# natir/yacrd

Measured on AMD Instinct MI355X. Metric: reads_per_sec_classified, higher is better.
Workload: dtype u32

## Files before the change

yacrd_amd/csrc/device_common.h:

```cpp
#pragma once
#include <hip/hip_runtime.h>
#include <stdint.h>

typedef uint32_t u32;
typedef uint64_t u64;
typedef int32_t i32;

namespace yk {

constexpr u32 kNoKey = 0xFFFFFFFFu;

typedef u32 u32x4_a8 __attribute__((ext_vector_type(4), aligned(8)));
template <bool NT = false>
__device__ __forceinline__ uint4 load_pair(const uint2 *p)
{
    u32x4_a8 q;
    if constexpr (NT) q = __builtin_nontemporal_load(reinterpret_cast<const u32x4_a8 *>(p));
    else q = *reinterpret_cast<const u32x4_a8 *>(p);
    return make_uint4(q.x, q.y, q.z, q.w);
}
typedef u64 u64x2_a8 __attribute__((ext_vector_type(2), aligned(8)));
__device__ __forceinline__ ulonglong2 load_extent(const u64 *p)
{
    const u64x2_a8 q = *reinterpret_cast<const u64x2_a8 *>(p);
    return make_ulonglong2(q.x, q.y);
}

struct OvlRec {
    u32 a, b, sa, ea, sb, eb;
};

constexpr u32 kKeyShift = 2;
constexpr u32 kMaxKeyPos = 0x3FFFFFFEu;
__device__ __forceinline__ void make_event_keys(uint2 v, u32 &ks, u32 &ke, u32 &bad, u32 &zero_len)
{
    const u32 z = (v.x == v.y) ? 2u : 0u;
    bad |= (v.x > v.y || v.y > kMaxKeyPos) ? 1u : 0u;
    zero_len += z;
    ks = ((v.x << kKeyShift) | 3u) - z;
    ke = (v.y << kKeyShift) + z;
}
constexpr u32 kNoFlag = 1u;

constexpr u32 kSmallEvents = 1024;
constexpr u32 kMedium1Events = 8192;
constexpr u32 kMedium2Events = 32768;
enum { CLS_R2 = 0, CLS_R4, CLS_R8, CLS_R16, CLS_H16, CLS_W2, CLS_W4, CLS_W8, CLS_W16, CLS_MED1,
       CLS_MED2, CLS_GENERAL, CLS_COUNT };

struct Counters {
    u32 n[16];
    u64 iv[16];
    u32 rej_small;
    u32 rej_med;
    u32 rej_big;
    u32 region_overflow;
    u32 scan_ticket;
    u32 ob_unsupported;
    u32 prefiltered;
    u32 over_med;
    u32 fb_med[2];
    u32 fb_big;
    u32 fbq_head[2];
    u32 fbq_done[2];
    u32 bs_chunks;
    u32 fused_gave_up;
    u64 total_regions;
    u32 fb_stream[2];
    alignas(128) u32 deferred;
    u64 deferred_iv;
};

struct SweepArgs {
    const u64 *off;
    const uint2 *iv;
    const u32 *len;
    const u32 *list;
    const u32 *list_n;
    const uint4 *rec;
    u32 first;
    u32 cov;
    u32 prefilter;
    uint2 *stage;
    u32 *counts;
    uint2 *closed;
    u32 *rej_list;
    u32 *rej_count;
    u32 *over_list;
    u32 *over_count;
    Counters *ctr;
};
constexpr u32 kDeferredMark = 0xFFFFFFFFu;
constexpr u32 kClosedForm = 0xFFFFFFFEu;

__device__ __forceinline__ u32 lane_id() { return threadIdx.x & 63u; }

#define YK_DPP_ZERO(v, ctrl, rm) (u32) __builtin_amdgcn_update_dpp(0, (int)(v), ctrl, rm, 0xF, true)
__device__ __forceinline__ u32 wave_incl_add(u32 v)
{
    v += YK_DPP_ZERO(v, 0x111, 0xF);
    v += YK_DPP_ZERO(v, 0x112, 0xF);
    v += YK_DPP_ZERO(v, 0x114, 0xF);
    v += YK_DPP_ZERO(v, 0x118, 0xF);
    v += YK_DPP_ZERO(v, 0x142, 0xA);
    v += YK_DPP_ZERO(v, 0x143, 0xC);
    return v;
}
__device__ __forceinline__ u32 wave_incl_max(u32 v)
{
    v = max(v, YK_DPP_ZERO(v, 0x111, 0xF));
    v = max(v, YK_DPP_ZERO(v, 0x112, 0xF));
    v = max(v, YK_DPP_ZERO(v, 0x114, 0xF));
    v = max(v, YK_DPP_ZERO(v, 0x118, 0xF));
    v = max(v, YK_DPP_ZERO(v, 0x142, 0xA));
    v = max(v, YK_DPP_ZERO(v, 0x143, 0xC));
    return v;
}
__device__ __forceinline__ u32 wave_shift_up1(u32 v) { return YK_DPP_ZERO(v, 0x138, 0xF); }
__device__ __forceinline__ u32 wave_min(u32 v)
{
#pragma unroll
    for (u32 d = 32; d > 0; d >>= 1) v = min(v, (u32)__shfl_xor(v, d, 64));
    return v;
}
__device__ __forceinline__ u32 wave_max(u32 v)
{
#pragma unroll
    for (u32 d = 32; d > 0; d >>= 1) v = max(v, (u32)__shfl_xor(v, d, 64));
    return v;
}
__device__ __forceinline__ u32 wave_or(u32 v)
{
#pragma unroll
    for (u32 d = 32; d > 0; d >>= 1) v |= (u32)__shfl_xor(v, d, 64);
    return v;
}

template <int T>
__device__ __forceinline__ u32 block_excl_add(u32 v, u32 *sc, u32 &total)
{
    u32 incl = wave_incl_add(v);
    if (T == 64) {
        total = __shfl(incl, 63, 64);
        return incl - v;
    }
    const u32 wid = threadIdx.x >> 6;
    if (lane_id() == 63) sc[wid] = incl;
    __syncthreads();
    u32 base = 0, tot = 0;
#pragma unroll
    for (u32 w = 0; w < T / 64; w++) {
        u32 x = sc[w];
        if (w < wid) base += x;
        tot += x;
// ... 89 lines not shown
```

yacrd_amd/csrc/finish_compact.h:

```cpp
#pragma once
#include "plan_compact.h"
#include "screen_reg.h"
#include "sweep_filtered.h"
#include "sweep_lds.h"
#include "sweep_wave.h"
#include "wave_ops.h"

namespace yk {

struct CompactArgs2 {
    SweepArgs sweep;
    u64 *scan_state;
    u32 n_reads;
    double not_cov;
    u64 *bad_offsets;
    uint2 *bad_regions;
    u64 region_cap;
    uint8_t *read_type;
    Counters *host_ctr;
};

constexpr int kFinishWaves = kScanBlock / 64;
#ifndef YK_FINISH_OCC
#define YK_FINISH_OCC 8
// ... 102 lines not shown
            for (i32 hi = (i32)bid - 1;; hi -= 64) {
                const i32 idx = hi - (i32)lane;
                u64 v, pre;
                for (;;) {
                    v = idx >= 0 ? __hip_atomic_load(&c.scan_state[idx], __ATOMIC_RELAXED, __HIP_MEMORY_SCOPE_AGENT)
                                 : kPre;
                    pre = __builtin_amdgcn_ballot_w64((v >> 62) == 2);
                    const u64 before = pre ? ((pre & (0 - pre)) - 1ull) : ~0ull;
                    if ((__builtin_amdgcn_ballot_w64((v >> 62) == 0) & before) == 0) break;
                    __builtin_amdgcn_s_sleep(1);
                }
                const u32 first_pre = pre ? (u32)__builtin_ctzll(pre) : 64u;
                u64 part = lane <= first_pre ? (v & kVal) : 0;
#pragma unroll
                for (int d = 32; d > 0; d >>= 1) part += __shfl_xor(part, d, 64);
                base += part;
                if (pre) break;
            }
        }
        if (lane == 0) {
            __hip_atomic_store(&c.scan_state[bid], kPre | (base + tot), __ATOMIC_RELAXED, __HIP_MEMORY_SCOPE_AGENT);
            s_base = base;
            if ((u64)(bid + 1) * kScanBlock >= c.n_reads) ctr->total_regions = base + tot;
        }
        if (c.host_ctr && (u64)(bid + 1) * kScanBlock >= c.n_reads) {
            const u64 total = (u64)__shfl((long long)(base + tot), 0, 64);
            const u32 *src = reinterpret_cast<const u32 *>(ctr);
            u32 *dst = reinterpret_cast<u32 *>(c.host_ctr);
            constexpr u32 kWords = (u32)(sizeof(Counters) / 4);
            for (u32 i = lane; i < kWords; i += 64u) {
                u32 w = __hip_atomic_load(&src[i], __ATOMIC_RELAXED, __HIP_MEMORY_SCOPE_AGENT);
                if (i == (u32)(offsetof(Counters, total_regions) / 4)) w = (u32)total;
                if (i == (u32)(offsetof(Counters, total_regions) / 4) + 1u) w = (u32)(total >> 32);
                if (i == (u32)(offsetof(Counters, region_overflow) / 4)) w = total > c.region_cap ? 1u : 0u;
                dst[i] = w;
            }
        }
    }
    __syncthreads();
    if (in) {
        const u64 dst = s_base + local;
        c.bad_offsets[r] = dst;
        if (r == c.n_reads - 1) c.bad_offsets[c.n_reads] = dst + g;

        u32 bad = 0;
        bool middle = false;
        const bool fits = dst + g <= c.region_cap;
        if (closed) {
            u32 k = 0;
            if (ab.x != 0u && fits) c.bad_regions[dst + k++] = make_uint2(0u, ab.x);
            if (ab.y != L && fits) c.bad_regions[dst + k] = make_uint2(ab.y, L);
            bad = ab.x + (L - ab.y);
        } else {
            const uint2 *slot = a.stage + (off_r + 2 * (u64)r);
            for (u32 k = 0; k < g; k++) {
                const uint2 v = slot[k];
                if (fits) c.bad_regions[dst + k] = v;
                bad += v.y - v.x;
                middle |= (v.x != 0u) & (v.y != L);
            }
        }
        if (!fits) atomicOr(&ctr->region_overflow, 1u);
        c.read_type[r] = (uint8_t)classify(bad, middle, L, c.not_cov);
    }
}


#ifndef YK_DEFER_SWEEP_OCC
#define YK_DEFER_SWEEP_OCC 6
#endif

template <int LANES, int WPB, int TABW = kScreenTabWords>
__device__ __forceinline__ bool filtered_turn(const SweepArgs &a, bool active, u32 r, u64 o, u32 n, u32 len, const LaneConst &lc)
{
    constexpr int K = 16;
    const u32 lane = lane_id(), lig = lane & (u32)(LANES - 1);
    const i32 c = (i32)min(a.cov, 0x3FFFFFFFu);
    const bool two = active && n >= 2u;
    const uint2 *src = two ? a.iv + o : reinterpret_cast<const uint2 *>(a.off);
    const u32 last2 = two ? n - 2u : 0u;
    uint4 v[K / 4];
#pragma unroll
    for (int j = 0; j < K / 4; j++) v[j] = load_pair(src + min(2u * (lig + (u32)LANES * j), last2));
    u32 smin = v[0].x, emax = v[0].y, smax = v[0].x;
    i32 tmin = 0x7FFFFFFF;
#pragma unroll
    for (int j = 0; j < K / 4; j++) {
        smin = min(smin, min(v[j].x, v[j].z));
        smax = max(smax, max(v[j].x, v[j].z));
        emax = max(emax, max(v[j].y, v[j].w));
        tmin = min(tmin, min((i32)(v[j].y - v[j].x), (i32)(v[j].w - v[j].z)));
    }
    const int last_addr = (int)((lane | (u32)(LANES - 1)) << 2);
    const u32 pmin = (u32)__builtin_amdgcn_ds_bpermute(last_addr, (int)gscan_min<LANES>(smin));
    const u32 pmax = (u32)__builtin_amdgcn_ds_bpermute(last_addr, (int)gscan_max<LANES>(emax));
    const bool irregular = !two || pmax > min(len, kMaxKeyPos) || smax > kMaxKeyPos || tmin < (i32)kScreenWindow;
    const bool girr = group_any<LANES>(__builtin_amdgcn_ballot_w64(irregular));
    const u32 n_eff = girr ? 0u : n;
    bool real0[K / 4], real1[K / 4];
#pragma unroll
    for (int j = 0; j < K / 4; j++) {
        const u32 i0 = 2u * (lig + (u32)LANES * j);
        real0[j] = i0 + 1u < n_eff;
        real1[j] = i0 < n_eff;
    }
    return filtered_group_sweep<LANES, WPB, TABW>(a, v, real0, real1, r, o, n, len, c, pmin, pmax, !girr, lc);
}
constexpr u32 kDeferShards = 256, kDeferShardStride = 16;
struct DeferList {
    u32 *list;
    u32 *count;
    u32 shard_cap;
};
constexpr int kMarkThreads = 1024, kMarkReads = 4 * kMarkThreads;
__global__ __launch_bounds__(kMarkThreads) void mark_list_kernel(const u32 *__restrict__ counts, u32 n_reads, DeferList dl)
{
    __shared__ u32 s_ids[kMarkReads];
    __shared__ u32 s_n, s_base;
    if (threadIdx.x == 0) s_n = 0;
    __syncthreads();
    const u64 r0 = (u64)blockIdx.x * kMarkReads + threadIdx.x * 4u;
    u32 g[4] = {0, 0, 0, 0};
    if (r0 + 4 <= n_reads) {
        const uint4 g4 = *reinterpret_cast<const uint4 *>(counts + r0);
        g[0] = g4.x, g[1] = g4.y, g[2] = g4.z, g[3] = g4.w;
    } else {
#pragma unroll
        for (int k = 0; k < 4; k++) g[k] = r0 + k < n_reads ? counts[r0 + k] : 0u;
    }
    u32 mine = 0;
#pragma unroll
    for (int k = 0; k < 4; k++) mine += g[k] == kDeferredMark ? 1u : 0u;
    if (__builtin_amdgcn_ballot_w64(mine != 0) != 0) {
        u32 incl = mine;
#pragma unroll
        for (int d = 1; d < 64; d <<= 1) {
            const u32 t = (u32)__shfl_up((int)incl, d, 64);
            if ((int)lane_id() >= d) incl += t;
        }
        u32 base = 0;
        if (lane_id() == 63u) base = atomicAdd(&s_n, incl);
        base = (u32)__shfl((int)base, 63, 64);
        u32 at = base + incl - mine;
#pragma unroll
        for (int k = 0; k < 4; k++)
            if (g[k] == kDeferredMark) s_ids[at++] = (u32)(r0 + k);
    }
    __syncthreads();
    const u32 n = s_n;
    if (n == 0) return;
    const u32 shard = blockIdx.x & (kDeferShards - 1u);
    if (threadIdx.x == 0) s_base = atomicAdd(dl.count + shard * kDeferShardStride, n);
    __syncthreads();
    const u32 b0 = s_base;
    for (u32 i = threadIdx.x; i < n; i += kMarkThreads)
        if (b0 + i < dl.shard_cap) dl.list[(size_t)shard * dl.shard_cap + b0 + i] = s_ids[i];
}

#ifndef YK_LIST_THREADS
#define YK_LIST_THREADS 512
#endif
#ifndef YK_LIST_OCC
#define YK_LIST_OCC YK_DEFER_SWEEP_OCC
#endif
constexpr int kListThreads = YK_LIST_THREADS;
__global__ __launch_bounds__(kListThreads, YK_LIST_OCC) void deferred_list_kernel(SweepArgs a, DeferList dl)
{
    constexpr u32 kWaves = kListThreads / 64;
    constexpr int kTabWords = 2 * (2 * kScreenWindow + 32) * 4;
    static_assert(kDeferShards <= (u32)kListThreads, "one thread per shard counter");
    __shared__ u32 s_pre[kDeferShards + 1];
    __shared__ u32 sc[kWaves + 1];
    __shared__ uint4 s_list[kListThreads];
    __shared__ unsigned short s_fb[kListThreads];
    __shared__ u32 s_nfb;
    __shared__ unsigned long long s_iv;
    const u32 tid = threadIdx.x, lane = lane_id(), wv = tid >> 6;
    u32 total;
    {
        const u32 cnt = tid < kDeferShards ? min(dl.count[tid * kDeferShardStride], dl.shard_cap) : 0u;
        const u32 ex = block_excl_add<kListThreads>(cnt, sc, total);
        if (tid < kDeferShards) s_pre[tid] = ex;
        if (tid == 0) s_pre[kDeferShards] = total;
    }
    const u32 per = (total + gridDim.x - 1u) / gridDim.x;
    const u32 lo = (u32)min((u64)total, (u64)blockIdx.x * per), hi = (u32)min((u64)total, (u64)lo + per);
    if (lo >= hi) return;
    const LaneConst lcf = make_lane_const(lane);
    if (tid == 0) s_iv = 0;
    for (u32 c0 = lo; c0 < hi; c0 += (u32)kListThreads) {
        __syncthreads();
        if (tid == 0) s_nfb = 0;
        const u32 e = c0 + tid, n_here = min((u32)kListThreads, hi - c0);
        if (e < hi) {
            u32 s = 0;
#pragma unroll
            for (u32 step = kDeferShards / 2; step > 0; step >>= 1)
                if (s_pre[s + step] <= e) s += step;
            const u32 r = dl.list[(size_t)s * dl.shard_cap + (e - s_pre[s])];
            const u64 o = a.off[r];
            const u32 n = (u32)(a.off[r + 1] - o);
            s_list[tid] = make_uint4(r, n, a.len[r], 0u);
            atomicAdd(&s_iv, (unsigned long long)n);
        }
        __syncthreads();
        for (u32 p0 = wv * 2u; p0 < n_here; p0 += kWaves * 2u) {
            const u32 p = p0 + (lane >> 5);
            const bool have = p < n_here;
            const uint4 q = s_list[have ? p : p0];
            const u64 o = a.off[q.x];
            const bool done = filtered_turn<32, (int)kWaves, kTabWords>(a, have, q.x, o, q.y, q.z, lcf);
            if (have && !done && (lane & 31u) == 31u) s_fb[atomicAdd(&s_nfb, 1u)] = (unsigned short)p;
        }
        __syncthreads();
        const u32 nfb = s_nfb;
        for (u32 i = wv; i < nfb; i += kWaves) {
            const uint4 q = s_list[s_fb[i]];
            const u64 o = a.off[q.x];
            if (q.y > 128u) finish_item<8>(a.off, a.iv, a.len, a.stage, a.counts, a.rej_list, a.rej_count, a.ctr, a.cov, q.x, o, q.y, q.z);
            else finish_item<4>(a.off, a.iv, a.len, a.stage, a.counts, a.rej_list, a.rej_count, a.ctr, a.cov, q.x, o, q.y, q.z);
        }
    }
    __syncthreads();
    if (tid == 0) {
        atomicAdd((unsigned long long *)&a.ctr->deferred_iv, s_iv);
        atomicAdd(&a.ctr->deferred, hi - lo);
    }
}

constexpr int kScanThreads = 1024;
template <int PER>
__global__ __launch_bounds__(kScanThreads) void scan_compact_kernel(CompactArgs2 c)
{
    constexpr int kScanPer = PER, kScanReads = kScanThreads * PER;
    static_assert(PER % 4 == 0 && kScanReads % kScanBlock == 0, "16-byte loads; the control block holds one scan word per 1024 reads: more than this kernel's workgroups use");
    __shared__ u32 sc[kScanThreads / 64];
    __shared__ u32 s_bid;
    __shared__ u64 s_base;
    const SweepArgs &a = c.sweep;
    Counters *ctr = a.ctr;
    if (threadIdx.x == 0) s_bid = atomicAdd(&ctr->scan_ticket, 1u);
    __syncthreads();
    const u32 bid = s_bid, lane = lane_id();
    const u64 r0 = (u64)bid * kScanReads + threadIdx.x * (u32)kScanPer;
    u32 g[kScanPer], L[kScanPer];
    uint2 ab[kScanPer];
    bool closed[kScanPer];
    const bool vec = r0 + kScanPer <= c.n_reads && (reinterpret_cast<uintptr_t>(a.len) & 15u) == 0;
    if (vec) {
#pragma unroll
        for (int q = 0; q < kScanPer / 4; q++) {
            const uint4 g4 = *reinterpret_cast<const uint4 *>(a.counts + r0 + 4 * q);
            const uint4 l4 = *reinterpret_cast<const uint4 *>(a.len + r0 + 4 * q);
            g[4 * q] = g4.x, g[4 * q + 1] = g4.y, g[4 * q + 2] = g4.z, g[4 * q + 3] = g4.w;
            L[4 * q] = l4.x, L[4 * q + 1] = l4.y, L[4 * q + 2] = l4.z, L[4 * q + 3] = l4.w;
        }
    } else {
#pragma unroll
        for (int k = 0; k < kScanPer; k++) {
            const bool in = r0 + k < c.n_reads;
            g[k] = in ? a.counts[r0 + k] : 0u;
            L[k] = in ? a.len[r0 + k] : 0u;
        }
    }
    bool any_closed = false;
#pragma unroll
    for (int k = 0; k < kScanPer; k++) {
        if (g[k] == kDeferredMark) g[k] = 0u;
        closed[k] = g[k] == kClosedForm;
        any_closed |= closed[k];
        ab[k] = make_uint2(0u, L[k]);
    }
    if (any_closed) {
        if (vec) {
#pragma unroll
            for (int q = 0; q < kScanPer / 2; q++) {
                const uint4 c0 = *reinterpret_cast<const uint4 *>(a.closed + r0 + 2 * q);
                if (closed[2 * q]) ab[2 * q] = make_uint2(c0.x, c0.y);
                if (closed[2 * q + 1]) ab[2 * q + 1] = make_uint2(c0.z, c0.w);
            }
        } else {
#pragma unroll
            for (int k = 0; k < kScanPer; k++)
                if (closed[k]) ab[k] = a.closed[r0 + k];
        }
    }
    u32 mine = 0;
#pragma unroll
    for (int k = 0; k < kScanPer; k++) {
        if (closed[k]) g[k] = (ab[k].x != 0u ? 1u : 0u) + (ab[k].y != L[k] ? 1u : 0u);
        mine += g[k];
    }
    u32 tot;
    u32 local = block_excl_add<kScanThreads>(mine, sc, tot);
    if (threadIdx.x < 64) {
        constexpr u64 kAgg = 1ull << 62, kPre = 2ull << 62, kVal = (1ull << 62) - 1;
        u64 base = 0;
        if (bid > 0) {
            if (lane == 0) __hip_atomic_store(&c.scan_state[bid], kAgg | tot, __ATOMIC_RELAXED, __HIP_MEMORY_SCOPE_AGENT);
            for (i32 hi = (i32)bid - 1;; hi -= 64) {
                const i32 idx = hi - (i32)lane;
                u64 v, pre;
                for (;;) {
                    v = idx >= 0 ? __hip_atomic_load(&c.scan_state[idx], __ATOMIC_RELAXED, __HIP_MEMORY_SCOPE_AGENT) : kPre;
                    pre = __builtin_amdgcn_ballot_w64((v >> 62) == 2);
                    const u64 before = pre ? ((pre & (0 - pre)) - 1ull) : ~0ull;
                    if ((__builtin_amdgcn_ballot_w64((v >> 62) == 0) & before) == 0) break;
                    __builtin_amdgcn_s_sleep(1);
                }
// ... 80 lines not shown
```

yacrd_amd/csrc/screen_reg.h:

```cpp
#pragma once
#include "device_common.h"
#include "wave_ops.h"

namespace yk {

#ifndef YK_SCREEN_WINDOW
#define YK_SCREEN_WINDOW 32
#endif
constexpr int kScreenWindow = YK_SCREEN_WINDOW;
constexpr int kScreenTabWords = (64 / 16) * (16 + 2 * kScreenWindow) * 4;
constexpr int kScreenTabWordsRows = (64 / 16) * (32 + 2 * kScreenWindow) * 4;
template <int WPB, int WORDS = kScreenTabWords>
__device__ __forceinline__ u32 *wave_screen_scratch()
{
    __shared__ __attribute__((aligned(16))) u32 s_tab[WPB][WORDS];
    return s_tab[threadIdx.x >> 6];
}

template <int LANES>
__device__ __forceinline__ bool group_any(u64 ballot)
{
    if (LANES == 64) return ballot != 0;
    return ((u32)(ballot >> (lane_id() & (u32)(64 - LANES))) & (u32)((1ull << (LANES & 63)) - 1ull)) != 0u;
}

struct HealthyRead {
    u32 a, b;
    i32 F, G;
};
#ifndef YK_SCREEN_SLIDES
#define YK_SCREEN_SLIDES 4
#endif
constexpr int kScreenSlides = YK_SCREEN_SLIDES;

template <int LANES, int WPB, bool SLID = false, int TABW = kScreenTabWords, int NB = LANES, int PAIRS = 4>
__device__ __forceinline__ bool healthy_screen(const uint4 (&v)[PAIRS], const bool (&real0)[PAIRS], const bool (&real1)[PAIRS],
                                               u32 len, i32 c, u32 pmin, u32 pmax, HealthyRead &hr, u32 P = 0, u32 Q = 0,
                                               u32 emin = 0, u32 smax = 0xFFFFFFFFu)
{
    constexpr int W = kScreenWindow, NBIN = 2 * W + NB, GROUPS = 64 / LANES, PER = W / LANES, ZPER = NBIN / LANES,
                  CPL = NB / LANES;
    constexpr u32 kEnd = 1u << 10, kField = kEnd - 1u;
    static_assert(W % LANES == 0 && PER >= 1 && W <= 64, "window bins per lane; a window index has six bits");
    static_assert(NB % LANES == 0 && NBIN % LANES == 0 && GROUPS * NBIN * 4 <= TABW, "scratch");
    static_assert(PAIRS * 2 * LANES <= 256, "a counter field has ten bits");
    const u32 lane = lane_id(), lig = lane & (u32)(LANES - 1), grp = lane / (u32)LANES;
    u32 *tab = wave_screen_scratch<WPB, TABW>() + grp * (u32)(NBIN * 4);
    uint4 *bins = reinterpret_cast<uint4 *>(tab);
    char *tb = reinterpret_cast<char *>(tab);

    const i32 bits = 32 - (i32)__builtin_clz(len | 1u) - ilog2c(NB) + (len != 0 ? 0 : -1);
    const u32 sh = (u32)max(bits, ilog2c(W));
    const u32 span = pmax - pmin, T = span - (u32)W;

#pragma unroll
    for (int q = 0; q < ZPER; q++) bins[lig + (u32)(LANES * q)] = make_uint4(0u, 0u, 0u, 0u);
    wave_lds_sync();

    const u32 cp = (lig & 3u) * 4u;
    u32 one = 1u, one_end = kEnd;
    if constexpr (!SLID) asm volatile("" : "+v"(one), "+v"(one_end));
    u32 ramp = 0;
    auto count = [&](u32 s, u32 e, bool real) {
        const u32 ds = s - pmin, dx = e - pmin;
        const u32 is = min(ds, (u32)W) + (ds >> sh);
        const u32 ie = (dx >> sh) + __builtin_elementwise_sub_sat(dx, T) + (u32)W;
        if constexpr (SLID) {
            const bool in_ramp = ds >= (u32)W && s < emin;
            ramp += (real && s >= pmin && in_ramp) ? 1u : 0u;
            if (real && s >= pmin && !in_ramp) atomicAdd(reinterpret_cast<u32 *>(tb + ((is << 4) + cp)), one);
            if (real && e <= pmax && !(e > smax && dx <= T)) atomicAdd(reinterpret_cast<u32 *>(tb + ((ie << 4) + cp)), one_end);
        } else if (real) {
            atomicAdd(reinterpret_cast<u32 *>(tb + ((is << 4) + cp)), one);
            atomicAdd(reinterpret_cast<u32 *>(tb + ((ie << 4) + cp)), one_end);
        }
    };
#pragma unroll
    for (int j = 0; j < PAIRS; j++) {
        count(v[j].x, v[j].y, real0[j]);
        count(v[j].z, v[j].w, real1[j]);
    }
    wave_lds_sync();

    u32 f[PER], fw = 0;
#pragma unroll
    for (int q = 0; q < PER; q++) {
        const u32 d = lig * (u32)PER + q;
        const u32 it = min((u32)(2 * W) - d + ((span - d) >> sh), (u32)(NBIN - 1));
        const uint4 h4 = bins[d], t4 = bins[it];
        f[q] = ((h4.x + h4.y + h4.z + h4.w) & kField) | ((t4.x + t4.y + t4.z + t4.w) & (kField << 10));
        fw += f[q];
    }
    u32 wb[CPL], w = 0;
#pragma unroll
    for (int q = 0; q < CPL; q++) {
        const uint4 c4 = bins[(u32)W + lig * (u32)CPL + q];
        wb[q] = (c4.x + c4.y + c4.z + c4.w) & ((kField << 10) | kField);
        w += wb[q];
    }
    const u32 fincl = gscan_add<LANES>(fw);
    u32 reached = 0;
    {
        const u32 k1 = (u32)min(c + 1, 0x1FF);
        u32 run = fincl - fw + (SLID ? ((512u - k1 + P) | ((512u - k1 + Q) << 10)) : (512u - k1) * (1u | kEnd));
#pragma unroll
        for (int q = 0; q < PER; q++) {
            run += f[q];
            reached += run & (0x200u | (0x200u << 10));
        }
    }
    const u32 cand = (((u32)PER - ((reached >> 9) & 7u)) << 20) | (((u32)PER - (reached >> 19)) << 26);
    const u32 wincl = gscan_add<LANES>(w | cand);
    u32 run = wincl - w, xl = 0xFFFFFFFFu;
#pragma unroll
    for (int q = 0; q < CPL; q++) {
        const u32 ex = run;
        run += wb[q];
        const i32 x = (i32)(ex & kField) - (i32)((run >> 10) & kField);
        xl = min(xl, (wb[q] & kField) != 0u ? (u32)(x + 0x10000) : 0xFFFFFFFFu);
    }
    const u32 xm = gscan_min<LANES>(xl);
    const i32 F = (i32)(fincl & kField) + (SLID ? (i32)P : 0), G = (i32)(fincl >> 10) + (SLID ? (i32)Q : 0);
    hr.F = F, hr.G = G;
    hr.a = pmin + ((wincl >> 20) & 63u);
    hr.b = pmax - (wincl >> 26);
    i32 open0 = F;
    if constexpr (SLID) open0 += (i32)gscan_add<LANES>(ramp);
    const bool deep = xm == 0xFFFFFFFFu || (i32)(xm - 0x10000u) + open0 > c;
    return deep && F > c && G > c;
}

struct VerdictsToGlobal {
    const SweepArgs &a;
    __device__ __forceinline__ void closed(u32 r, u32 ra, u32 rb, u32 len) const
    {
        if (ra != 0 || rb != len) a.closed[r] = make_uint2(ra, rb);
        else a.counts[r] = 0;
        if (a.prefilter == 2) atomicAdd(&a.ctr->prefiltered, 1u);
    }
    __device__ __forceinline__ void deferred(u32 r) const { a.counts[r] = kDeferredMark; }
};

template <int ITEMS>
struct ReadsKnown {
    u64 o[ITEMS];
    u32 n[ITEMS], len[ITEMS];
};

template <int LANES, int ITEMS, bool WIDE, int WPB = 1, int K = 16, int NB = LANES, bool NT = (ITEMS >= 2),
          int TABW = kScreenTabWords, class Sink>
__device__ __forceinline__ void screen_reads(const SweepArgs &a, const u32 (&r)[ITEMS], const bool (&active)[ITEMS], const Sink &sink,
                                             const ReadsKnown<ITEMS> *known = nullptr)
{
    static_assert(K % 4 == 0, "a lane takes its intervals in pairs");
    const u32 lane = lane_id(), lig = lane & (u32)(LANES - 1);
    const i32 c = (i32)min(a.cov, 0x3FFFFFFFu);
    u32 n[ITEMS], len[ITEMS];
    u64 o[ITEMS];
#pragma unroll
    for (int t = 0; t < ITEMS; t++) {
        o[t] = 0, n[t] = 0, len[t] = 0;
        if (known) {
            if (active[t]) o[t] = known->o[t], n[t] = known->n[t], len[t] = known->len[t];
        } else if (active[t]) {
            const ulonglong2 oo = load_extent(a.off + r[t]);
            o[t] = oo.x;
            n[t] = (u32)(oo.y - oo.x);
            len[t] = a.len[r[t]];
        }
    }
    uint4 v[ITEMS][K / 4];
#pragma unroll
    for (int t = 0; t < ITEMS; t++) {
        const bool two = n[t] >= 2u;
        const uint2 *src = two ? a.iv + o[t] : reinterpret_cast<const uint2 *>(a.off);
        const u32 last2 = two ? n[t] - 2u : 0u;
#pragma unroll
        for (int j = 0; j < K / 4; j++)
            v[t][j] = load_pair<NT>(src + min(2u * (lig + (u32)LANES * j), last2));
    }
#pragma unroll
    for (int t = 0; t < ITEMS; t++) {
        if (t > 0 && __builtin_amdgcn_ballot_w64(active[t]) == 0) break;
        const u32 len_c = min(len[t], kMaxKeyPos);
        u32 smin = v[t][0].x, emax = v[t][0].y, smax = v[t][0].x;
        i32 tmin = 0x7FFFFFFF;
#pragma unroll
        for (int j = 0; j < K / 4; j++) {
            smin = min(smin, min(v[t][j].x, v[t][j].z));
            smax = max(smax, max(v[t][j].x, v[t][j].z));
            emax = max(emax, max(v[t][j].y, v[t][j].w));
            tmin = min(tmin, min((i32)(v[t][j].y - v[t][j].x), (i32)(v[t][j].w - v[t][j].z)));
        }
        const int last_addr = (int)((lane | (u32)(LANES - 1)) << 2);
        const u32 pmin = (u32)__builtin_amdgcn_ds_bpermute(last_addr, (int)gscan_min<LANES>(smin));
        const u32 pmax = (u32)__builtin_amdgcn_ds_bpermute(last_addr, (int)gscan_max<LANES>(emax));
        const bool irregular = n[t] < 2u || pmax > len_c || smax > kMaxKeyPos || tmin < (i32)kScreenWindow;
        const bool girr = group_any<LANES>(__builtin_amdgcn_ballot_w64(irregular));
        const u32 n_eff = girr ? 0u : n[t];
        bool real0[K / 4], real1[K / 4];
#pragma unroll
        for (int j = 0; j < K / 4; j++) {
            const u32 i0 = 2u * (lig + (u32)LANES * j);
            real0[j] = i0 + 1u < n_eff;
            real1[j] = i0 < n_eff;
        }
        HealthyRead hr;
        bool healthy = healthy_screen<LANES, WPB, false, TABW, NB>(v[t], real0, real1, len[t], c, pmin, pmax, hr) && !girr;
        if constexpr (kScreenSlides > 0 && WIDE) {
            auto state_of = [&](bool nd, const HealthyRead &h) {
// ... 70 lines not shown
```

yacrd_amd/csrc/sweep_filtered.h:

```cpp
#pragma once
#include "screen_reg.h"
#include "wave_ops.h"

namespace yk {

constexpr int kFilteredCap = 128;
constexpr u32 kFilteredPad = 0xFFFFFFFFu;
static_assert(kScreenWindow * 4 >= kFilteredCap, "the keys live in the tail window's bins");

template <int LANES, int WPB, int TABW = kScreenTabWords>
__device__ __forceinline__ bool filtered_group_sweep(const SweepArgs &a, const uint4 (&v)[4], const bool (&real0)[4], const bool (&real1)[4],
                                                     u32 r, u64 o, u32 n, u32 len, i32 c, u32 pmin, u32 pmax, bool want, const LaneConst &lc)
{
    constexpr int NB = LANES, W = kScreenWindow, NBIN = 2 * W + NB, K = kFilteredCap / LANES;
    constexpr u32 kEnd = 1u << 10, kField = kEnd - 1u;
    static_assert(LANES == 16 || LANES == 32, "group masks are 32-bit");
    const u32 lane = lane_id(), lig = lane & (u32)(LANES - 1), grp = lane / (u32)LANES;
    const int last_addr = (int)((lane | (u32)(LANES - 1)) << 2);
    const u32 gshift = lane & (u32)(64 - LANES);
    constexpr u32 gmask = LANES == 32 ? 0xFFFFFFFFu : 0xFFFFu;
    auto to_group = [&](u32 x) { return (u32)__builtin_amdgcn_ds_bpermute(last_addr, (int)x); };
    auto group_bits = [&](bool b) { return (u32)(__builtin_amdgcn_ballot_w64(b) >> gshift) & gmask; };
    static_assert((64 / LANES) * NBIN * 4 <= TABW, "scratch");
    u32 *tab = wave_screen_scratch<WPB, TABW>() + grp * (u32)(NBIN * 4);
    uint4 *bins = reinterpret_cast<uint4 *>(tab);
    u32 *info = tab;
    u32 *keys = tab + (u32)((W + NB) * 4);
    const bool last = lig == (u32)(LANES - 1);

    HealthyRead hr;
    bool r0[4], r1[4];
#pragma unroll
    for (int j = 0; j < 4; j++) r0[j] = real0[j] && want, r1[j] = real1[j] && want;
    const bool healthy = healthy_screen<LANES, WPB, false, TABW>(v, r0, r1, len, c, pmin, pmax, hr);
    const u32 hF = to_group((u32)min(max(hr.F, 0), 1023) | ((hr.G > c && want && (i32)n > c) ? 0x400u : 0u) | (healthy ? 0x800u : 0u));
    const i32 F = (i32)(hF & 1023u);
    bool ok = (hF & 0x400u) != 0u && F > c;
    const bool is_healthy = ok && (hF & 0x800u) != 0u;
    if (__builtin_amdgcn_ballot_w64(ok) == 0) return false;
    const u32 ga = to_group(hr.a), gb = to_group(hr.b);

    const i32 bits = 32 - (i32)__builtin_clz(len | 1u) - ilog2c(NB) + (len != 0 ? 0 : -1);
    const u32 sh = (u32)max(bits, ilog2c(W));
    const u32 span = pmax - pmin, T = span - (u32)W, iT = T >> sh;
    const uint4 c4 = bins[(u32)W + lig];
    const u32 w = (c4.x + c4.y + c4.z + c4.w) & ((kField << 10) | kField);
    const i32 S = (i32)(w & kField), E = (i32)(w >> 10);
    const u32 wincl = gscan_add<LANES>(w), wex = wincl - w;
    const i32 D = F + (i32)(wex & kField) - (i32)(wex >> 10);
    const bool inside = lig <= iT;
    const bool unsafe = ok && !is_healthy && inside && S + E > 0 && D - E <= c;
    const u32 mu = group_bits(unsafe), me = group_bits(inside && E > 0);
    const u32 higher = ((mu | me) >> lig) >> 1;
    const bool kept = unsafe || (ok && inside && E > 0 && higher != 0u && (((mu >> lig) >> 1) >> __builtin_ctz(higher | 0x80000000u)) & 1u);
    const u32 km = group_bits(kept);
    const u32 pack = kept ? (u32)(S + E) + ((u32)(S - E) << 16) : 0u;
    const u32 pincl = gscan_add<LANES>(pack), pex = pincl - pack;
    const u32 m = to_group(pincl) & 0xFFFFu;
    ok = ok && m <= (u32)kFilteredCap;
    if (__builtin_amdgcn_ballot_w64(ok) == 0) return false;
    wave_lds_sync();
    *reinterpret_cast<uint2 *>(info + 2u * lig) = make_uint2(pex & 0xFFFFu, (u32)(D - ((i32)pex >> 16)));
    {
        uint4 *kp = reinterpret_cast<uint4 *>(keys + lig * (u32)K);
#pragma unroll
        for (int q = 0; q < K / 4; q++) kp[q] = make_uint4(kFilteredPad, kFilteredPad, kFilteredPad, kFilteredPad);
    }
    wave_lds_sync();

    auto put = [&](u32 s, u32 e, bool real) {
        const u32 ds = s - pmin, dx = e - pmin;
        const u32 bs = ds >> sh, be = dx >> sh;
        if (real && ok && ds >= (u32)W && ((km >> bs) & 1u)) keys[atomicAdd(info + 2u * bs, 1u)] = (s << kKeyShift) | 3u;
        if (real && ok && dx <= T && ((km >> be) & 1u)) keys[atomicAdd(info + 2u * be, 1u)] = e << kKeyShift;
    };
#pragma unroll
    for (int j = 0; j < 4; j++) {
        put(v[j].x, v[j].y, r0[j]);
        put(v[j].z, v[j].w, r1[j]);
    }
    wave_lds_sync();
    u32 x[K];
    {
        const uint4 *kp = reinterpret_cast<const uint4 *>(keys + lig * (u32)K);
#pragma unroll
        for (int q = 0; q < K / 4; q++) {
            const uint4 t = kp[q];
            x[4 * q] = t.x, x[4 * q + 1] = t.y, x[4 * q + 2] = t.z, x[4 * q + 3] = t.w;
        }
    }
    bitonic_sort<LANES, K, 2>(x, lc);

    i32 corr[K];
    u32 dl = 0;
#pragma unroll
    for (int q = 0; q < K; q++) {
        const bool real = x[q] != kFilteredPad;
        const u32 blk = real ? (((x[q] >> kKeyShift) - pmin) >> sh) : 0u;
        corr[q] = (i32)info[2u * blk + 1u];
        dl += real ? ((x[q] & 1u) << 1) - 1u : 0u;
    }
    const i32 depth_in = (i32)(gscan_add<LANES>(dl) - dl);
    u32 mf = 0, ml = 0;
    {
        i32 d = depth_in;
#pragma unroll
        for (int q = 0; q < K; q++) {
            const u32 key = x[q];
            const bool real = key != kFilteredPad, is_s = (key & 1u) != 0u, gt = d + corr[q] > c;
            mf = (real && !is_s && gt) ? key : mf;
            ml = (real && is_s && !gt) ? key : ml;
            d += real ? (is_s ? 1 : -1) : 0;
        }
    }
    const u32 mf_incl = gscan_max<LANES>(mf), ml_incl = gscan_max<LANES>(ml);
    const u32 mf_in = gshift_up1<LANES>(mf_incl), ml_in = gshift_up1<LANES>(ml_incl);
    u32 cnt = 0, fb = 0, fe = 0;
    bool orphan = false;
    {
        u32 tc = mf_in, cml = ml_in;
        i32 d = depth_in;
#pragma unroll
        for (int q = 0; q < K; q++) {
            const u32 key = x[q];
            const bool real = key != kFilteredPad, is_s = (key & 1u) != 0u, gt = d + corr[q] > c;
            const bool fl = real && !is_s && gt, low = real && is_s && !gt;
            const bool close = fl && cml > tc;
            cnt += close ? 1u : 0u;
            fb = close ? tc : fb;
            fe = close ? cml : fe;
            orphan |= low && tc == 0u;
            tc = fl ? key : tc;
            cml = low ? key : cml;
            d += real ? (is_s ? 1 : -1) : 0;
        }
    }
    ok = ok && group_bits(orphan) == 0u;
    if (__builtin_amdgcn_ballot_w64(ok) == 0) return false;
    const u32 g0 = ga != 0u ? 1u : 0u;
    const u32 cincl = gscan_add<LANES>(cnt);
    if (ok && (cnt != 0u || last)) {
        uint2 *slot = a.stage + (o + 2 * (u64)r);
        u32 pos = g0 + cincl - cnt;
        if (cnt == 1u) {
            slot[pos] = make_uint2(fb >> kKeyShift, fe >> kKeyShift);
        } else if (cnt > 1u) {
            u32 tc = mf_in, cml = ml_in;
            i32 d = depth_in;
#pragma unroll
            for (int q = 0; q < K; q++) {
                const u32 key = x[q];
                const bool real = key != kFilteredPad, is_s = (key & 1u) != 0u, gt = d + corr[q] > c;
                const bool fl = real && !is_s && gt, low = real && is_s && !gt;
                if (fl && cml > tc) slot[pos++] = make_uint2(tc >> kKeyShift, cml >> kKeyShift);
                tc = fl ? key : tc;
                cml = low ? key : cml;
                d += real ? (is_s ? 1 : -1) : 0;
            }
        }
        if (last) {
            u32 g = g0 + cincl;
            if (ga != 0u) slot[0] = make_uint2(0u, ga);
            if (ml_incl > mf_incl) slot[g++] = make_uint2(mf_incl >> kKeyShift, ml_incl >> kKeyShift);
            if (gb != len) slot[g++] = make_uint2(gb, len);
            a.counts[r] = g;
        }
    }
    return ok;
}

}
```

yacrd_amd/engine.py:

```python
import ctypes
import os
import subprocess
from collections import namedtuple

import numpy as np

_HERE = os.path.dirname(os.path.abspath(__file__))
_LIB = os.path.join(_HERE, "lib", "libyacrd_hip.so")

NOT_BAD, CHIMERIC, NOT_COVERED = 0, 1, 2
TYPE_NAMES = {NOT_BAD: "NotBad", CHIMERIC: "Chimeric", NOT_COVERED: "NotCovered"}
F_FORCE_GENERAL = 1
F_FORCE_LDS_SORT = 2
F_WAVE_ONLY = 8
F_NO_HALVES = 16
F_TIMING_FULL = 32
F_NO_PREDICTION = 64
F_NO_PREFILTER = 256
F_COUNT_PREFILTERED = 512
F_NO_TIMING = 1024
F_BLOCKING_WAIT = 2048
F_NO_DEFER = 4096
F_ALWAYS_DEFER = 8192
F_TIMING_SAMPLED = 32768
# ... 496 lines not shown
            keep = ctypes.create_string_buffer(bytes(path_or_bytes), len(path_or_bytes))
            addr, n = ctypes.addressof(keep), len(path_or_bytes)
        rc = self._lib.yacrd_engine_ingest_report_mem(self._h, addr, n, int(n_threads), float(not_coverage), ctypes.byref(res),
                                                      ctypes.byref(rd), ctypes.byref(st))
        del keep
        return self._ingested(rc, res, rd, st)

    def _ingested(self, rc, res, rd, st):
        if rc == E_FALLBACK:
            raise NeedsHostParser(self._lib.yacrd_last_error().decode())
        _check(self._lib, rc)
        R = int(rd.n_reads)
        lengths = np.ctypeslib.as_array(rd.lengths, shape=(R,)).copy() if R else np.zeros(0, np.uint32)
        off = np.ctypeslib.as_array(rd.name_off, shape=(R + 1,)).copy()
        blob = ctypes.string_at(rd.names, int(off[-1])) if R else b""
        names = [blob[int(off[i]):int(off[i + 1])].decode("utf-8", "surrogateescape") for i in range(R)]
        stats = {n: getattr(st, n) for n, _ in _IngestStats._fields_}
        self._lib.yacrd_reads_free(ctypes.byref(rd))
        return _take(self._lib, res), names, lengths, stats

    def _report_table(self, names, lengths, result):
        if names is None and lengths is None and result is None:
            return None, None
        if names is None or lengths is None or result is None:
            raise ValueError("names, lengths and result: all three, or none for the table the last ingest left on the device")
        blobs = [n if isinstance(n, bytes) else n.encode("utf-8", "surrogateescape") for n in names]
        R = len(blobs)
        off = np.zeros(R + 1, np.uint64)
        if blobs:
            off[1:] = np.cumsum([len(b) for b in blobs], dtype=np.uint64)
        blob = ctypes.create_string_buffer(b"".join(blobs), int(off[-1]) + 1)
        lens = np.ascontiguousarray(lengths, dtype=np.uint32)
        bo = np.ascontiguousarray(result.bad_offsets, dtype=np.uint64)
        br = np.ascontiguousarray(result.bad_regions, dtype=np.uint32).reshape(-1)
        rt = np.ascontiguousarray(result.read_type, dtype=np.uint8)
        if lens.shape != (R,) or bo.shape != (R + 1,) or rt.shape != (R,) or (R and br.size != 2 * int(bo[-1])):
            raise ValueError("the report table's arrays do not fit one another")
        if br.size == 0:
            br = np.zeros(2, np.uint32)
        if R == 0:
            lens, rt = np.zeros(1, np.uint32), np.zeros(1, np.uint8)
        t = _ReportTable(R, off.ctypes.data, ctypes.addressof(blob), lens.ctypes.data, bo.ctypes.data, br.ctypes.data, rt.ctypes.data)
        return ctypes.byref(t), (t, off, blob, lens, bo, br, rt)

    def _report_written(self, rc, st):
        if rc == E_FALLBACK:
            raise NeedsHostParser(self._lib.yacrd_last_error().decode())
        _check(self._lib, rc)
        self.report_write_stats = {n: getattr(st, n) for n, _ in _ReportWriteStats._fields_}
        return self.report_write_stats

    def write_report(self, out_path, names=None, lengths=None, result=None):
        t, keep = self._report_table(names, lengths, result)
        st = _ReportWriteStats()
        rc = self._lib.yacrd_engine_write_report(self._h, t, os.fsencode(out_path), ctypes.byref(st))
        del keep
        return self._report_written(rc, st)

    def report_text(self, names=None, lengths=None, result=None):
        t, keep = self._report_table(names, lengths, result)
        st = _ReportWriteStats()
        out, n_out = ctypes.c_void_p(), ctypes.c_uint64()
        rc = self._lib.yacrd_engine_write_report_mem(self._h, t, ctypes.byref(out), ctypes.byref(n_out), ctypes.byref(st))
        del keep
        self._report_written(rc, st)
        try:
            return ctypes.string_at(out.value, int(n_out.value)) if n_out.value else b""
        finally:
            self._lib.yacrd_edit_text_free(out)

    def debug_sort_pairs(self, keys, vals, key_bound):
        keys = np.array(keys, dtype=np.uint64)
        vals = np.array(vals, dtype=np.uint32)
        _check(self._lib, self._lib.yacrd_debug_sort_pairs(self._h, keys.ctypes.data, vals.ctypes.data, keys.shape[0], int(key_bound)))
        return keys, vals

    def debug_counters(self):
        class _Counters(ctypes.Structure):
            _fields_ = [("n", ctypes.c_uint32 * 16), ("iv", ctypes.c_uint64 * 16), ("rej_small", ctypes.c_uint32),
                        ("rej_med", ctypes.c_uint32), ("rej_big", ctypes.c_uint32), ("region_overflow", ctypes.c_uint32),
                        ("scan_ticket", ctypes.c_uint32), ("ob_unsupported", ctypes.c_uint32), ("prefiltered", ctypes.c_uint32),
                        ("over_med", ctypes.c_uint32), ("fb_med", ctypes.c_uint32 * 2), ("fb_big", ctypes.c_uint32),
                        ("fbq_head", ctypes.c_uint32 * 2), ("fbq_done", ctypes.c_uint32 * 2), ("bs_chunks", ctypes.c_uint32),
                        ("fused_gave_up", ctypes.c_uint32), ("total_regions", ctypes.c_uint64)]
        c = _Counters()
        self._lib.yacrd_debug_last_counters.restype = ctypes.c_uint64
        self._lib.yacrd_debug_last_counters.argtypes = [ctypes.c_void_p, ctypes.c_void_p, ctypes.c_uint64]
        self._lib.yacrd_debug_last_counters(self._h, ctypes.byref(c), ctypes.sizeof(c))
        out = {}
        for n, _ in _Counters._fields_:
            v = getattr(c, n)
            out[n] = list(v) if hasattr(v, "__len__") else int(v)
        return out

    def _type_table(self, names, read_type):
        blobs = [n if isinstance(n, bytes) else n.encode("utf-8", "surrogateescape") for n in names]
        off = np.zeros(len(blobs) + 1, np.uint64)
        if blobs:
            off[1:] = np.cumsum([len(b) for b in blobs], dtype=np.uint64)
        blob = ctypes.create_string_buffer(b"".join(blobs), int(off[-1]) + 1)
        types = np.ascontiguousarray(read_type, dtype=np.uint8)
        if types.shape != (len(blobs),):
            raise ValueError("read_type: one type per name")
        tt = _TypeTable(len(blobs), off.ctypes.data, ctypes.addressof(blob), types.ctypes.data)
        return tt, (off, blob, types)

    def _edited(self, rc, st):
        if rc == E_FALLBACK:
            raise NeedsHostParser(self._lib.yacrd_last_error().decode())
        _check(self._lib, rc)
        self.edit_stats = {n: getattr(st, n) for n, _ in _EditStats._fields_}
        return self.edit_stats

    def edit_overlaps(self, op, src, out_path, names, read_type, fmt=0, n_threads=0):
        tt, keep = self._type_table(names, read_type)
        st = _EditStats()
        rc = self._lib.yacrd_engine_edit_overlaps(self._h, int(op), os.fsencode(src), os.fsencode(out_path), int(fmt), int(n_threads),
                                                  ctypes.byref(tt), ctypes.byref(st))
        del keep
        return self._edited(rc, st)

    def edit_overlaps_text(self, op, text, names, read_type, fmt):
        tt, keep = self._type_table(names, read_type)
        st = _EditStats()
        buf = ctypes.create_string_buffer(bytes(text), len(text) + 1)
        out, n_out = ctypes.c_void_p(), ctypes.c_uint64()
        rc = self._lib.yacrd_engine_edit_overlaps_mem(self._h, int(op), ctypes.addressof(buf), len(text), int(fmt), ctypes.byref(tt),
                                                      ctypes.byref(out), ctypes.byref(n_out), ctypes.byref(st))
        del keep
        self._edited(rc, st)
        try:
            return ctypes.string_at(out.value, int(n_out.value)) if n_out.value else b""
        finally:
            self._lib.yacrd_edit_text_free(out)

    def edit_overlaps_gzip(self, op, text, names, read_type, fmt, out_path=None):
        tt, keep = self._type_table(names, read_type)
        st, gs = _EditStats(), _GzipStats()
        buf = np.frombuffer(text, dtype=np.uint8)
        n = int(buf.size)
        addr = ctypes.c_void_p(buf.ctypes.data if n else None)
        out, n_out = ctypes.c_void_p(), ctypes.c_uint64()
        if out_path is None:
            rc = self._lib.yacrd_engine_edit_overlaps_gzip_mem(self._h, int(op), addr, n, int(fmt), ctypes.byref(tt),
                                                               ctypes.byref(out), ctypes.byref(n_out), ctypes.byref(st), ctypes.byref(gs))
        else:
            rc = self._lib.yacrd_engine_edit_overlaps_gzip_file(self._h, int(op), addr, n, int(fmt), ctypes.byref(tt),
                                                                os.fsencode(out_path), ctypes.byref(st), ctypes.byref(gs))
        del keep, buf
        self._edited(rc, st)
        self.gzip_stats = {f: getattr(gs, f) for f, _ in _GzipStats._fields_}
        if out_path is not None:
            return self.edit_stats, self.gzip_stats
        try:
            return ctypes.string_at(out.value, int(n_out.value))
        finally:
            self._lib.yacrd_edit_text_free(out)

    def gzip(self, data):
        data = bytes(data)
        st = _GzipStats()
        out, n_out = ctypes.c_void_p(), ctypes.c_uint64()
        buf = ctypes.create_string_buffer(data, len(data) + 1)
        _check(self._lib, self._lib.yacrd_engine_gzip_mem(self._h, ctypes.addressof(buf), len(data), ctypes.byref(out), ctypes.byref(n_out),
                                                          ctypes.byref(st)))
        self.gzip_stats = {f: getattr(st, f) for f, _ in _GzipStats._fields_}
        try:
            return ctypes.string_at(out.value, int(n_out.value))
        finally:
            self._lib.yacrd_edit_text_free(out)

    def gzip_writer(self, out_path, segment_bytes=0, n_buffers=0):
        return GzipWriter(self, out_path, segment_bytes, n_buffers)
# ... 291 lines not shown
```

Before: 3.299 billion.

## Unify filtered screen windows so more reads finish on the fast path

Replaces the separate healthy and filtered checks with a unified window map in healthy_screen. It records head ends and tail starts plus a refuse flag, and relaxes the irregular-read test so more reads stay on the register-screen path instead of falling back. Reads with no kept bins now write their bad regions straight away and skip the LDS key sort. It also adds a deferred_whole counter with a matching layout for the Python debug struct. The correctness conditions become more intricate, with zero-length and orphan handling, so misclassifying edge reads is a risk.

```diff
diff --git a/yacrd_amd/csrc/device_common.h b/yacrd_amd/csrc/device_common.h
--- a/yacrd_amd/csrc/device_common.h
+++ b/yacrd_amd/csrc/device_common.h
@@ -69,7 +69,9 @@
     u32 fb_stream[2];
     alignas(128) u32 deferred;
     u64 deferred_iv;
+    u32 deferred_whole;
 };
+static_assert(sizeof(Counters) == 512, "the block goes home as 512 bytes; yacrd_amd/engine.py::debug_counters mirrors the layout");
 
 struct SweepArgs {
     const u64 *off;
diff --git a/yacrd_amd/csrc/finish_compact.h b/yacrd_amd/csrc/finish_compact.h
--- a/yacrd_amd/csrc/finish_compact.h
+++ b/yacrd_amd/csrc/finish_compact.h
@@ -208,11 +208,11 @@
     uint4 v[K / 4];
 #pragma unroll
     for (int j = 0; j < K / 4; j++) v[j] = load_pair(src + min(2u * (lig + (u32)LANES * j), last2));
-    u32 smin = v[0].x, emax = v[0].y, smax = v[0].x;
+    u32 smin = 0xFFFFFFFFu, emax = v[0].y, smax = v[0].x;
     i32 tmin = 0x7FFFFFFF;
 #pragma unroll
     for (int j = 0; j < K / 4; j++) {
-        smin = min(smin, min(v[j].x, v[j].z));
+        smin = min(smin, min(v[j].y != 0u ? v[j].x : 0xFFFFFFFFu, v[j].w != 0u ? v[j].z : 0xFFFFFFFFu));
         smax = max(smax, max(v[j].x, v[j].z));
         emax = max(emax, max(v[j].y, v[j].w));
         tmin = min(tmin, min((i32)(v[j].y - v[j].x), (i32)(v[j].w - v[j].z)));
@@ -220,7 +220,7 @@
     const int last_addr = (int)((lane | (u32)(LANES - 1)) << 2);
     const u32 pmin = (u32)__builtin_amdgcn_ds_bpermute(last_addr, (int)gscan_min<LANES>(smin));
     const u32 pmax = (u32)__builtin_amdgcn_ds_bpermute(last_addr, (int)gscan_max<LANES>(emax));
-    const bool irregular = !two || pmax > min(len, kMaxKeyPos) || smax > kMaxKeyPos || tmin < (i32)kScreenWindow;
+    const bool irregular = !two || len > kMaxKeyPos || pmax > len || smax > kMaxKeyPos || tmin < 0 || pmax - pmin < (u32)(2 * kScreenWindow);
     const bool girr = group_any<LANES>(__builtin_amdgcn_ballot_w64(irregular));
     const u32 n_eff = girr ? 0u : n;
     bool real0[K / 4], real1[K / 4];
@@ -299,7 +299,7 @@
     __shared__ u32 sc[kWaves + 1];
     __shared__ uint4 s_list[kListThreads];
     __shared__ unsigned short s_fb[kListThreads];
-    __shared__ u32 s_nfb;
+    __shared__ u32 s_nfb, s_whole;
     __shared__ unsigned long long s_iv;
     const u32 tid = threadIdx.x, lane = lane_id(), wv = tid >> 6;
     u32 total;
@@ -313,7 +313,7 @@
     const u32 lo = (u32)min((u64)total, (u64)blockIdx.x * per), hi = (u32)min((u64)total, (u64)lo + per);
     if (lo >= hi) return;
     const LaneConst lcf = make_lane_const(lane);
-    if (tid == 0) s_iv = 0;
+    if (tid == 0) s_iv = 0, s_whole = 0;
     for (u32 c0 = lo; c0 < hi; c0 += (u32)kListThreads) {
         __syncthreads();
         if (tid == 0) s_nfb = 0;
@@ -340,6 +340,7 @@
         }
         __syncthreads();
         const u32 nfb = s_nfb;
+        if (tid == 0) s_whole += nfb;
         for (u32 i = wv; i < nfb; i += kWaves) {
             const uint4 q = s_list[s_fb[i]];
             const u64 o = a.off[q.x];
@@ -351,6 +352,7 @@
     if (tid == 0) {
         atomicAdd((unsigned long long *)&a.ctr->deferred_iv, s_iv);
         atomicAdd(&a.ctr->deferred, hi - lo);
+        if (s_whole) atomicAdd(&a.ctr->deferred_whole, s_whole);
     }
 }
 
diff --git a/yacrd_amd/csrc/screen_reg.h b/yacrd_amd/csrc/screen_reg.h
--- a/yacrd_amd/csrc/screen_reg.h
+++ b/yacrd_amd/csrc/screen_reg.h
@@ -28,16 +28,21 @@
     u32 a, b;
     i32 F, G;
 };
+struct UnifiedWindows {
+    u32 head_ends, tail_starts;
+    bool refuse;
+};
 #ifndef YK_SCREEN_SLIDES
 #define YK_SCREEN_SLIDES 4
 #endif
 constexpr int kScreenSlides = YK_SCREEN_SLIDES;
 
-template <int LANES, int WPB, bool SLID = false, int TABW = kScreenTabWords, int NB = LANES, int PAIRS = 4>
+template <int LANES, int WPB, bool SLID = false, int TABW = kScreenTabWords, int NB = LANES, int PAIRS = 4, bool UNIFIED = false>
 __device__ __forceinline__ bool healthy_screen(const uint4 (&v)[PAIRS], const bool (&real0)[PAIRS], const bool (&real1)[PAIRS],
                                                u32 len, i32 c, u32 pmin, u32 pmax, HealthyRead &hr, u32 P = 0, u32 Q = 0,
-                                               u32 emin = 0, u32 smax = 0xFFFFFFFFu)
-{
+                                               u32 emin = 0, u32 smax = 0xFFFFFFFFu, UnifiedWindows *uw = nullptr)
+{
+    static_assert(!(UNIFIED && SLID), "the unified map's windows do not slide");
     constexpr int W = kScreenWindow, NBIN = 2 * W + NB, GROUPS = 64 / LANES, PER = W / LANES, ZPER = NBIN / LANES,
                   CPL = NB / LANES;
     constexpr u32 kEnd = 1u << 10, kField = kEnd - 1u;
@@ -70,6 +75,11 @@
             ramp += (real && s >= pmin && in_ramp) ? 1u : 0u;
             if (real && s >= pmin && !in_ramp) atomicAdd(reinterpret_cast<u32 *>(tb + ((is << 4) + cp)), one);
             if (real && e <= pmax && !(e > smax && dx <= T)) atomicAdd(reinterpret_cast<u32 *>(tb + ((ie << 4) + cp)), one_end);
+        } else if constexpr (UNIFIED) {
+            if (real && e != 0u) {
+                atomicAdd(reinterpret_cast<u32 *>(tb + (((is + __builtin_elementwise_sub_sat(ds, T)) << 4) + cp)), one);
+                atomicAdd(reinterpret_cast<u32 *>(tb + (((ie - (u32)W + min(dx, (u32)W)) << 4) + cp)), one_end);
+            }
         } else if (real) {
             atomicAdd(reinterpret_cast<u32 *>(tb + ((is << 4) + cp)), one);
             atomicAdd(reinterpret_cast<u32 *>(tb + ((ie << 4) + cp)), one_end);
@@ -83,6 +93,7 @@
     wave_lds_sync();
 
     u32 f[PER], fw = 0;
+    [[maybe_unused]] u32 g[PER], gw = 0;
 #pragma unroll
     for (int q = 0; q < PER; q++) {
         const u32 d = lig * (u32)PER + q;
@@ -90,6 +101,12 @@
         const uint4 h4 = bins[d], t4 = bins[it];
         f[q] = ((h4.x + h4.y + h4.z + h4.w) & kField) | ((t4.x + t4.y + t4.z + t4.w) & (kField << 10));
         fw += f[q];
+        if constexpr (UNIFIED) {
+            g[q] = (((h4.x + h4.y + h4.z + h4.w) >> 10) & kField) | (((t4.x + t4.y + t4.z + t4.w) & kField) << 10);
+            const u32 he0 = g[q] & kField;
+            if (q == 0 && lig == 0u && c >= 1 && (f[q] & kField) > he0) f[q] -= he0, fw -= he0, g[q] -= he0;
+            gw += g[q];
+        }
     }
     u32 wb[CPL], w = 0;
 #pragma unroll
@@ -99,6 +116,22 @@
         w += wb[q];
     }
     const u32 fincl = gscan_add<LANES>(fw);
+    if constexpr (UNIFIED) {
+        const u32 gincl = gscan_add<LANES>(gw);
+        u32 run_f = fincl - fw, run_g = gincl - gw;
+        bool refuse = false;
+#pragma unroll
+        for (int q = 0; q < PER; q++) {
+            const i32 cs = (i32)(run_f & kField), te = (i32)(run_f >> 10);
+            run_f += f[q], run_g += g[q];
+            const i32 ce = (i32)(run_g & kField), ts = (i32)(run_g >> 10);
+            const u32 hs = f[q] & kField, he = g[q] & kField, tn = f[q] >> 10, tl = g[q] >> 10;
+            refuse |= (hs + he) != 0u && cs - ce <= c && (he != 0u || cs > c);
+            refuse |= te - ts <= c && (tl != 0u || (tn != 0u && te > c));
+        }
+        uw->refuse = refuse;
+        uw->head_ends = gincl & kField, uw->tail_starts = gincl >> 10;
+    }
     u32 reached = 0;
     {
         const u32 k1 = (u32)min(c + 1, 0x1FF);
@@ -126,6 +159,7 @@
     hr.b = pmax - (wincl >> 26);
     i32 open0 = F;
     if constexpr (SLID) open0 += (i32)gscan_add<LANES>(ramp);
+    if constexpr (UNIFIED) return F > c && G > c;
     const bool deep = xm == 0xFFFFFFFFu || (i32)(xm - 0x10000u) + open0 > c;
     return deep && F > c && G > c;
 }
diff --git a/yacrd_amd/csrc/sweep_filtered.h b/yacrd_amd/csrc/sweep_filtered.h
--- a/yacrd_amd/csrc/sweep_filtered.h
+++ b/yacrd_amd/csrc/sweep_filtered.h
@@ -29,14 +29,14 @@
     const bool last = lig == (u32)(LANES - 1);
 
     HealthyRead hr;
+    UnifiedWindows uw;
     bool r0[4], r1[4];
 #pragma unroll
     for (int j = 0; j < 4; j++) r0[j] = real0[j] && want, r1[j] = real1[j] && want;
-    const bool healthy = healthy_screen<LANES, WPB, false, TABW>(v, r0, r1, len, c, pmin, pmax, hr);
-    const u32 hF = to_group((u32)min(max(hr.F, 0), 1023) | ((hr.G > c && want && (i32)n > c) ? 0x400u : 0u) | (healthy ? 0x800u : 0u));
-    const i32 F = (i32)(hF & 1023u);
-    bool ok = (hF & 0x400u) != 0u && F > c;
-    const bool is_healthy = ok && (hF & 0x800u) != 0u;
+    const bool both = healthy_screen<LANES, WPB, false, TABW, LANES, 4, true>(v, r0, r1, len, c, pmin, pmax, hr, 0, 0, 0, 0xFFFFFFFFu, &uw);
+    const u32 hF = to_group((u32)min(max(hr.F, 0), 1023) | ((both && want) ? 0x400u : 0u) | (uw.head_ends << 12) | (uw.tail_starts << 22));
+    const i32 F = (i32)(hF & 1023u), HE = (i32)((hF >> 12) & 1023u);
+    bool ok = (hF & 0x400u) != 0u && group_bits(uw.refuse) == 0u;
     if (__builtin_amdgcn_ballot_w64(ok) == 0) return false;
     const u32 ga = to_group(hr.a), gb = to_group(hr.b);
 
@@ -44,13 +44,15 @@
     const u32 sh = (u32)max(bits, ilog2c(W));
     const u32 span = pmax - pmin, T = span - (u32)W, iT = T >> sh;
     const uint4 c4 = bins[(u32)W + lig];
-    const u32 w = (c4.x + c4.y + c4.z + c4.w) & ((kField << 10) | kField);
+    const bool inside = lig <= iT;
+    const u32 w = inside ? (c4.x + c4.y + c4.z + c4.w) & ((kField << 10) | kField) : 0u;
     const i32 S = (i32)(w & kField), E = (i32)(w >> 10);
     const u32 wincl = gscan_add<LANES>(w), wex = wincl - w;
-    const i32 D = F + (i32)(wex & kField) - (i32)(wex >> 10);
-    const bool inside = lig <= iT;
-    const bool unsafe = ok && !is_healthy && inside && S + E > 0 && D - E <= c;
+    const i32 D = F - HE + (i32)(wex & kField) - (i32)(wex >> 10);
+    ok = ok && (u32)F + (hF >> 22) + (to_group(wincl) & kField) >= 2u;
+    const bool unsafe = ok && inside && S + E > 0 && D - E <= c;
     const u32 mu = group_bits(unsafe), me = group_bits(inside && E > 0);
+    ok = ok && !(HE > 0 && (mu & ((mu | me) & (0u - (mu | me)))) != 0u);
     const u32 higher = ((mu | me) >> lig) >> 1;
     const bool kept = unsafe || (ok && inside && E > 0 && higher != 0u && (((mu >> lig) >> 1) >> __builtin_ctz(higher | 0x80000000u)) & 1u);
     const u32 km = group_bits(kept);
@@ -59,6 +61,16 @@
     const u32 m = to_group(pincl) & 0xFFFFu;
     ok = ok && m <= (u32)kFilteredCap;
     if (__builtin_amdgcn_ballot_w64(ok) == 0) return false;
+    if (__builtin_amdgcn_ballot_w64(ok && m != 0u) == 0) {
+        if (ok && last) {
+            uint2 *slot = a.stage + (o + 2 * (u64)r);
+            u32 g = 0;
+            if (ga != 0u) slot[g++] = make_uint2(0u, ga);
+            if (gb != len) slot[g++] = make_uint2(gb, len);
+            a.counts[r] = g;
+        }
+        return ok;
+    }
     wave_lds_sync();
     *reinterpret_cast<uint2 *>(info + 2u * lig) = make_uint2(pex & 0xFFFFu, (u32)(D - ((i32)pex >> 16)));
     {
@@ -68,11 +80,15 @@
     }
     wave_lds_sync();
 
+    bool zero_kept = false;
     auto put = [&](u32 s, u32 e, bool real) {
         const u32 ds = s - pmin, dx = e - pmin;
         const u32 bs = ds >> sh, be = dx >> sh;
-        if (real && ok && ds >= (u32)W && ((km >> bs) & 1u)) keys[atomicAdd(info + 2u * bs, 1u)] = (s << kKeyShift) | 3u;
-        if (real && ok && dx <= T && ((km >> be) & 1u)) keys[atomicAdd(info + 2u * be, 1u)] = e << kKeyShift;
+        const bool ks = real && ok && ds - (u32)W <= T - (u32)W && ((km >> bs) & 1u);
+        const bool ke = real && ok && dx - (u32)W <= T - (u32)W && ((km >> be) & 1u);
+        if (ks) keys[atomicAdd(info + 2u * bs, 1u)] = (s << kKeyShift) | 3u;
+        if (ke) keys[atomicAdd(info + 2u * be, 1u)] = e << kKeyShift;
+        zero_kept |= ks && s == e;
     };
 #pragma unroll
     for (int j = 0; j < 4; j++) {
@@ -135,7 +151,7 @@
             d += real ? (is_s ? 1 : -1) : 0;
         }
     }
-    ok = ok && group_bits(orphan) == 0u;
+    ok = ok && group_bits(orphan || zero_kept) == 0u;
     if (__builtin_amdgcn_ballot_w64(ok) == 0) return false;
     const u32 g0 = ga != 0u ? 1u : 0u;
     const u32 cincl = gscan_add<LANES>(cnt);
diff --git a/yacrd_amd/engine.py b/yacrd_amd/engine.py
--- a/yacrd_amd/engine.py
+++ b/yacrd_amd/engine.py
@@ -602,13 +602,18 @@
                         ("scan_ticket", ctypes.c_uint32), ("ob_unsupported", ctypes.c_uint32), ("prefiltered", ctypes.c_uint32),
                         ("over_med", ctypes.c_uint32), ("fb_med", ctypes.c_uint32 * 2), ("fb_big", ctypes.c_uint32),
                         ("fbq_head", ctypes.c_uint32 * 2), ("fbq_done", ctypes.c_uint32 * 2), ("bs_chunks", ctypes.c_uint32),
-                        ("fused_gave_up", ctypes.c_uint32), ("total_regions", ctypes.c_uint64)]
+                        ("fused_gave_up", ctypes.c_uint32), ("total_regions", ctypes.c_uint64),
+                        ("fb_stream", ctypes.c_uint32 * 2), ("_pad", ctypes.c_uint8 * 104),
+                        ("deferred", ctypes.c_uint32), ("deferred_iv", ctypes.c_uint64), ("deferred_whole", ctypes.c_uint32)]
+        assert _Counters.deferred.offset == 384 and _Counters.deferred_whole.offset == 400
         c = _Counters()
         self._lib.yacrd_debug_last_counters.restype = ctypes.c_uint64
         self._lib.yacrd_debug_last_counters.argtypes = [ctypes.c_void_p, ctypes.c_void_p, ctypes.c_uint64]
         self._lib.yacrd_debug_last_counters(self._h, ctypes.byref(c), ctypes.sizeof(c))
         out = {}
         for n, _ in _Counters._fields_:
+            if n.startswith("_"):
+                continue
             v = getattr(c, n)
             out[n] = list(v) if hasattr(v, "__len__") else int(v)
         return out
```

Measured after the change: 3.158 billion. 0.957x the previous value.
